# AdrienWohrer/diff-icp

Measured on AMD Instinct MI355X. Metric: PSR iterations/sec + kernel-sum HBM GB/s, 100k-pt 3D, 1/2/4/8 MI355X, higher is better.
Workload: dtype f32

## Files before the change

diff-icp_amd/csrc/lddmm_sym_pk.hpp:

```cpp
#pragma once
#include "lddmm_sym.hpp"
#include "packed.hpp"

namespace dicp {

template <int D>
struct CutBox {
  float lo[D], hi[D];
};
__device__ __forceinline__ float cut_uniform(float x) {
  return __builtin_bit_cast(float, __builtin_amdgcn_readfirstlane(__builtin_bit_cast(int, x)));
}
__device__ __forceinline__ float nan_min(float a, float b) { return (b < a || b != b) ? b : a; }
__device__ __forceinline__ float nan_max(float a, float b) { return (b > a || b != b) ? b : a; }
template <int D>
__device__ __forceinline__ void cut_load(const float* __restrict__ boxes, int s, CutBox<D>& b) {
#pragma unroll
  for (int d = 0; d < D; ++d) {
    b.lo[d] = boxes[(int64_t)s * (2 * D) + d];
    b.hi[d] = boxes[(int64_t)s * (2 * D) + D + d];
  }
}
template <int D, int N>
__device__ __forceinline__ void cut_row_box(const float* __restrict__ boxes, int s0, int nB, CutBox<D>& r) {
#pragma unroll
  for (int d = 0; d < D; ++d) r.lo[d] = __builtin_huge_valf(), r.hi[d] = -__builtin_huge_valf();
#pragma unroll
  for (int k = 0; k < N; ++k) {
    if (s0 + k >= nB) break;
    CutBox<D> b;
    cut_load<D>(boxes, s0 + k, b);
#pragma unroll
    for (int d = 0; d < D; ++d) r.lo[d] = nan_min(r.lo[d], b.lo[d]), r.hi[d] = nan_max(r.hi[d], b.hi[d]);
  }
#pragma unroll
  for (int d = 0; d < D; ++d) r.lo[d] = cut_uniform(r.lo[d]), r.hi[d] = cut_uniform(r.hi[d]);
}
template <int D, int N>
__device__ __forceinline__ unsigned cut_mask(const float* __restrict__ boxes, const CutBox<D>& r, int B, int nB,
                                             float T) {
  unsigned m = 0;
#pragma unroll
  for (int h = 0; h < N; ++h) {
    const int s = B * N + h;
    if (s >= nB) break;
    CutBox<D> c;
    cut_load<D>(boxes, s, c);
    float gap2 = 0.f;
#pragma unroll
    for (int d = 0; d < D; ++d) {
      const float a = r.lo[d] - c.hi[d], b = c.lo[d] - r.hi[d];
      float g = a > b ? a : b;
      g = g > 0.f ? g : 0.f;
      gap2 = fmaf(g, g, gap2);
    }
    if (gap2 > T) m |= 1u << h;
  }
  return (unsigned)__builtin_amdgcn_readfirstlane((int)m);
}

template <int D>
__global__ __launch_bounds__(256) void pair_boxes_kernel(Args a, int64_t M, int nB, float* __restrict__ boxes) {
  const int s = (int)blockIdx.x * 4 + (int)(threadIdx.x >> 6), l = threadIdx.x & 63;
  if (s >= nB) return;
  const int64_t i = (int64_t)s * kCutTile + l;
  float lo[D], hi[D];
  bool bad = false;
  if (i < M) {
    float c[D];
    ld_coord<D>(a, a.c0, i, c);
#pragma unroll
    for (int d = 0; d < D; ++d) {
      lo[d] = hi[d] = c[d];
      bad = bad || !(fabsf(c[d]) < __builtin_huge_valf());
    }
  } else {
#pragma unroll
    for (int d = 0; d < D; ++d) lo[d] = __builtin_huge_valf(), hi[d] = -__builtin_huge_valf();
  }
#pragma unroll
  for (int off = 32; off > 0; off >>= 1) {
#pragma unroll
    for (int d = 0; d < D; ++d) {
      lo[d] = fminf(lo[d], __shfl_xor(lo[d], off, 64));
      hi[d] = fmaxf(hi[d], __shfl_xor(hi[d], off, 64));
    }
  }
  const bool anybad = __any(bad);
  if (l < 2 * D) {
    float v = 0.f;
#pragma unroll
    for (int d = 0; d < D; ++d) {
      if (l == d) v = lo[d];
      if (l == D + d) v = hi[d];
    }
    boxes[(int64_t)s * (2 * D) + l] = anybad ? __builtin_nanf("") : v;
  }
}
template <int D>
int launch_pair_boxes(const Args& a, int64_t M, float* boxes, hipStream_t st) {
  if (M <= 0) return DICP_OK;
  const int nB = cut_tiles(M);
  pair_boxes_kernel<D><<<dim3((unsigned)((nB + 3) / 4)), dim3(256), 0, st>>>(a, M, nB, boxes);
  return check_launch("pair_boxes");
}

#ifndef DICP_SYMBWD_SCALAR_CT
#define DICP_SYMBWD_SCALAR_CT 1
#endif
template <int D, bool GQ = true, bool B0 = false, bool GT = true, bool RAW = false>
struct SymBwdPk {
  using S = SymBwd<D>;
  static constexpr int W = GQ ? 2 * D : D;
  static constexpr int kMaxWaves = 4;
#ifndef DICP_SYMBWD_PK_REC3
#define DICP_SYMBWD_PK_REC3 1
#endif
  static constexpr bool kRec3 = DICP_SYMBWD_PK_REC3 && D == 3;
  static constexpr int kPlanes = kRec3 ? 5 : S::CW;
  static constexpr bool kDupW = kRec3;
  __host__ __device__ static constexpr int slot(int i) { return kRec3 ? (i / 3) * 4 + i % 3 : i; }
  __device__ static void colvec(const float* rec, f2* cv) {
#pragma unroll
    for (int i = 0; i < 5 * D; ++i) cv[i] = splat(rec[i]);
    if constexpr (kDupW) {
#pragma unroll
      for (int m = 0; m < 5; ++m) cv[3 * m + 2] = f2{rec[3 * m + 2], rec[4 * S::CW + m]};
    }
  }
  struct Prm {
    float gt, c;
    float nc, s2;
  };
  __device__ static Prm params(const Args& a, const Scal& sc) {
    const float cs = sc.aux1 / a.scale;
    return Prm{sc.aux0 * cs, cs, sc.nc, RAW ? sc.s : kS2};
  }
  struct Row2 {
    f2 q[D], p[D], b[D], ia_a[D], gp[D];
  };
  __device__ static void pack(const typename S::Row& r0, const typename S::Row& r1, Row2& r) {
// ... 66 lines not shown
      t.cKzb = (splat(c) * zb) * t.K;
    } else {
      f2 zb = t.z[0] * (r.b[0] - bj[0]);
#pragma unroll
      for (int d = 1; d < D; ++d) zb = pk_fma(t.z[d], r.b[d] - bj[d], zb);
      t.cKzb = (splat(c) * zb) * t.K;
    }
  }
  __device__ static void pair_row(const Prm& prm, const Row2& r, const float* rec, f2* acc) {
    const float gt = prm.gt;
    f2 cv[5 * D];
    colvec(rec, cv);
    Shared t;
    shared_terms(prm, r, cv, t);
    const f2* pj = cv + D;
    const f2* aj = cv + 2 * D;
#pragma unroll
    for (int d = 0; d < D; ++d) {
      const f2 ka = GT ? pk_fma(splat(-gt), t.z[d], aj[d]) : aj[d];
      if constexpr (B0)
        acc[d] = pk_fma(t.K, ka, acc[d]);
      else
        acc[d] = pk_fma(t.cKzb, pj[d], pk_fma(t.K, ka, acc[d]));
      if constexpr (GQ) acc[D + d] = pk_fma(t.K, pk_fma(t.w, t.z[d], -t.u[d]), acc[D + d]);
    }
  }
  __device__ static void pair_sym(const Prm& prm, const Row2& r, const float* rec, f2* acc, float* ct) {
    const float gt = prm.gt;
    f2 cv[5 * D];
    colvec(rec, cv);
    Shared t;
    shared_terms(prm, r, cv, t);
    const f2* pj = cv + D;
    const f2* aj = cv + 2 * D;
    if constexpr (!GT) {
#pragma unroll
      for (int d = 0; d < D; ++d) {
        if constexpr (B0)
          acc[d] = pk_fma(t.K, aj[d], acc[d]);
        else
          acc[d] = pk_fma(t.cKzb, pj[d], pk_fma(t.K, aj[d], acc[d]));
#if DICP_SYMBWD_SCALAR_CT
        float cg = fmaf(t.K.x, r.ia_a[d].x, t.K.y * r.ia_a[d].y);
        if constexpr (!B0) cg = fmaf(t.cKzb.x, r.p[d].x, fmaf(t.cKzb.y, r.p[d].y, cg));
        ct[d] = cg;
#else
        const f2 cg = B0 ? t.K * r.ia_a[d] : pk_fma(t.cKzb, r.p[d], t.K * r.ia_a[d]);
        ct[d] = cg.x + cg.y;
#endif
        if constexpr (GQ) {
          const f2 e = pk_fma(t.w, t.z[d], -t.u[d]);
#if DICP_SYMBWD_SCALAR_CT
          acc[D + d] = pk_fma(t.K, e, acc[D + d]);
          ct[D + d] = -fmaf(t.K.x, e.x, t.K.y * e.y);
#else
          const f2 Ke = t.K * e;
          acc[D + d] = acc[D + d] + Ke;
          ct[D + d] = -(Ke.x + Ke.y);
#endif
        }
      }
      return;
    }
#pragma unroll
    for (int d = 0; d < D; ++d) {
      const f2 tt = pk_fma(splat(gt), t.z[d], r.ia_a[d]);
      if constexpr (B0) {
        acc[d] = pk_fma(t.K, pk_fma(splat(-gt), t.z[d], aj[d]), acc[d]);
        const f2 cg = t.K * tt;
        ct[d] = cg.x + cg.y;
      } else {
        acc[d] = pk_fma(t.cKzb, pj[d], pk_fma(t.K, pk_fma(splat(-gt), t.z[d], aj[d]), acc[d]));
        const f2 cg = pk_fma(t.cKzb, r.p[d], t.K * tt);
        ct[d] = cg.x + cg.y;
      }
      if constexpr (GQ) {
        const f2 e = pk_fma(t.w, t.z[d], -t.u[d]);
        const f2 Ke = t.K * e;
        acc[D + d] = acc[D + d] + Ke;
        ct[D + d] = -(Ke.x + Ke.y);
      }
    }
  }
  __device__ static void pair_sym4(const Prm& prm, const Row2& r0, const Row2& r1, const float* rec,
                                   f2* acc0, f2* acc1, float* ct) {
    const float gt = prm.gt;
    f2 cv[5 * D];
    colvec(rec, cv);
    Shared t0, t1;
    shared_terms(prm, r0, cv, t0);
    shared_terms(prm, r1, cv, t1);
    const f2* pj = cv + D;
    const f2* aj = cv + 2 * D;
#pragma unroll
    for (int d = 0; d < D; ++d) {
      const f2 ka0 = GT ? pk_fma(splat(-gt), t0.z[d], aj[d]) : aj[d];
      const f2 ka1 = GT ? pk_fma(splat(-gt), t1.z[d], aj[d]) : aj[d];
      const f2 tt0 = GT ? pk_fma(splat(gt), t0.z[d], r0.ia_a[d]) : r0.ia_a[d];
      const f2 tt1 = GT ? pk_fma(splat(gt), t1.z[d], r1.ia_a[d]) : r1.ia_a[d];
      f2 cg;
      if constexpr (B0) {
        acc0[d] = pk_fma(t0.K, ka0, acc0[d]);
        acc1[d] = pk_fma(t1.K, ka1, acc1[d]);
        cg = pk_fma(t1.K, tt1, t0.K * tt0);
      } else {
        acc0[d] = pk_fma(t0.cKzb, pj[d], pk_fma(t0.K, ka0, acc0[d]));
        acc1[d] = pk_fma(t1.cKzb, pj[d], pk_fma(t1.K, ka1, acc1[d]));
        cg = pk_fma(t1.cKzb, r1.p[d], pk_fma(t1.K, tt1, pk_fma(t0.cKzb, r0.p[d], t0.K * tt0)));
      }
      ct[d] = cg.x + cg.y;
      if constexpr (GQ) {
        const f2 e0 = pk_fma(t0.w, t0.z[d], -t0.u[d]);
        const f2 e1 = pk_fma(t1.w, t1.z[d], -t1.u[d]);
        const f2 Ke0 = t0.K * e0;
        acc0[D + d] = acc0[D + d] + Ke0;
        acc1[D + d] = pk_fma(t1.K, e1, acc1[D + d]);
        const f2 cs = pk_fma(t1.K, e1, Ke0);
        ct[D + d] = -(cs.x + cs.y);
      }
    }
  }
};

template <class P, class = void>
struct rec_layout {
  static constexpr int kPlanes = P::S::CW;
  static constexpr bool kDupW = false;
  __host__ __device__ static constexpr int slot(int i) { return i; }
};
template <class P>
struct rec_layout<P, std::void_t<decltype(P::kPlanes)>> {
  static constexpr int kPlanes = P::kPlanes;
  static constexpr bool kDupW = P::kDupW;
  __host__ __device__ static constexpr int slot(int i) { return P::slot(i); }
};
template <class P>
__host__ __device__ constexpr int plane_width(int m) {
  if (rec_layout<P>::kDupW) return 4;
  int w = 0;
  for (int i = 0; i < P::S::kUsed; ++i)
    if (rec_layout<P>::slot(i) / 4 == m && rec_layout<P>::slot(i) % 4 + 1 > w) w = rec_layout<P>::slot(i) % 4 + 1;
  return w;
}

#ifndef DICP_SYMBWD_PK_WMIN
#define DICP_SYMBWD_PK_WMIN 1
#endif
#ifndef DICP_SYMBWD_PK_WMAX
#define DICP_SYMBWD_PK_WMAX 4
#endif
#ifndef DICP_SYMBWD_PK_PREFETCH
#define DICP_SYMBWD_PK_PREFETCH 0
#endif
#ifndef DICP_SYMBWD_PK_UNROLL
#define DICP_SYMBWD_PK_UNROLL 2
#endif
template <class P>
__device__ __forceinline__ void sym_pk_body(Args a, Scal sc, int64_t M, int nG, int L,
                                            float* __restrict__ slab, int64_t slot_stride, int qoff,
                                            int qstride, unsigned bx, unsigned by) {
  using S = typename P::S;
  using LY = rec_layout<P>;
  constexpr int CW = S::CW, NP = LY::kPlanes, W = P::W;
  __shared__ float4 planes[2][NP][kSymG];
  __shared__ float colacc[kSymQ][kSymG][W];
  if (sc.dev0 != nullptr) sc.aux0 = sc.dev0[0];
  const typename P::Prm prm = P::params(a, sc);

// ... 108 lines not shown
#pragma unroll
        for (int k = 0; k < W; ++k) cacc[k] = rol1(cacc[k]);
      } else if (diag) {
#pragma unroll 2
        for (int k2 = 0; k2 < 64; ++k2) {
          const int col = h * 64 + ((l + k2) & 63);
          float rec[4 * CW + NP];
          ldrec(col, rec);
          P::pair_row(prm, row, rec, racc);
        }
      }
#pragma unroll
      for (int k = 0; k < W; ++k) colacc[wv][h * 64 + l][k] = cacc[k];
    }
    __syncthreads();
    if (tid < kSymG) {
      const int64_t j = (int64_t)B * kSymG + tid;
      if (j < M) {
        float* dst = slab + (int64_t)Q * slot_stride + j * W;
#pragma unroll
        for (int k = 0; k < W; ++k)
          dst[k] = ((colacc[0][tid][k] + colacc[1][tid][k]) + colacc[2][tid][k]) + colacc[3][tid][k];
      }
    }
    __syncthreads();
    buf ^= 1;
  }
#pragma unroll
  for (int r = 0; r < 2; ++r) {
    if (!rv[r]) continue;
    float* dst = slab + (int64_t)(Q + 1 + kc) * slot_stride + ri[r] * W;
#pragma unroll
    for (int k = 0; k < W; ++k) dst[k] = r == 0 ? racc[k].x : racc[k].y;
  }
}

#ifndef DICP_SYMBWD4_UNROLL
#define DICP_SYMBWD4_UNROLL 2
#endif
#ifndef DICP_SYMBWD4_WMIN
#define DICP_SYMBWD4_WMIN 1
#endif
template <class P, int DC = 0>
__device__ __forceinline__ void sym_pk4_body(Args a, Scal sc, int64_t M, int nG, int L,
                                             float* __restrict__ slab, int64_t slot_stride, int qoff,
                                             int qstride, unsigned bx, unsigned by,
                                             const float* __restrict__ boxes = nullptr, float T = 0.f) {
  using S = typename P::S;
  using LY = rec_layout<P>;
  constexpr int G = kSymG4;
  constexpr int CW = S::CW, NP = LY::kPlanes, W = P::W;
  __shared__ float4 planes[2][NP][G];
  __shared__ float colacc[kSymQ][G][W];
  if (sc.dev0 != nullptr) sc.aux0 = sc.dev0[0];
  const typename P::Prm prm = P::params(a, sc);

  const int Q = qoff + qstride * (int)by, kc = (int)bx;
  const int B0 = kSymQ * Q + kc * L;
  if (B0 >= nG) return;
  const int B1 = min(B0 + L, nG);
  const int tid = threadIdx.x, wv = tid >> 6, l = tid & 63;
  const int A = kSymQ * Q + wv;

  typename P::Row2 row[2];
  int64_t ri[4];
  bool rv[4];
  {
    typename S::Row r4[4];
#pragma unroll
    for (int r = 0; r < 4; ++r) {
      ri[r] = (int64_t)A * G + r * 64 + l;
      rv[r] = A < nG && ri[r] < M;
      S::load_row(a, sc, rv[r] ? ri[r] : 0, rv[r], r4[r]);
    }
    P::pack(r4[0], r4[1], row[0]);
    P::pack(r4[2], r4[3], row[1]);
  }
  f2 racc[2][W];
#pragma unroll
  for (int h = 0; h < 2; ++h)
#pragma unroll
    for (int k = 0; k < W; ++k) racc[h][k] = splat(0.f);

  CutBox<(DC > 0 ? DC : 1)> rbox;
  const int nB = cut_tiles(M);
  if constexpr (DC > 0) cut_row_box<DC, G / 64>(boxes, __builtin_amdgcn_readfirstlane(A) * (G / 64), nB, rbox);

  auto stage = [&](int B, int buf) {
    const int64_t j = (int64_t)B * G + tid;
    float rec[4 * CW], ph[4 * NP];
    S::load_col(a, sc, j < M ? j : 0, j < M, rec);
#pragma unroll
    for (int k = 0; k < 4 * NP; ++k) ph[k] = 0.f;
#pragma unroll
    for (int i = 0; i < S::kUsed; ++i) ph[LY::slot(i)] = rec[i];
    if constexpr (LY::kDupW) {
#pragma unroll
      for (int m = 0; m < NP; ++m) ph[4 * m + 3] = ph[4 * m + 2];
    }
#pragma unroll
    for (int m = 0; m < NP; ++m)
      planes[buf][m][tid] = make_float4(ph[4 * m], ph[4 * m + 1], ph[4 * m + 2], ph[4 * m + 3]);
  };

  int buf = 0;
  auto ldrec = [&](int col, float* rec) {
    float ph[4 * NP];
#pragma unroll
    for (int m = 0; m < NP; ++m) {
      const int w = plane_width<P>(m);
      const float* src = reinterpret_cast<const float*>(&planes[buf][m][col]);
      if (w == 4) {
        const float4 v = *reinterpret_cast<const float4*>(src);
        ph[4 * m] = v.x, ph[4 * m + 1] = v.y, ph[4 * m + 2] = v.z, ph[4 * m + 3] = v.w;
      } else if (w == 3) {
        const float3 v = *reinterpret_cast<const float3*>(src);
        ph[4 * m] = v.x, ph[4 * m + 1] = v.y, ph[4 * m + 2] = v.z, ph[4 * m + 3] = 0.f;
      } else if (w == 2) {
        const float2 v = *reinterpret_cast<const float2*>(src);
        ph[4 * m] = v.x, ph[4 * m + 1] = v.y, ph[4 * m + 2] = ph[4 * m + 3] = 0.f;
      } else {
        ph[4 * m] = src[0], ph[4 * m + 1] = ph[4 * m + 2] = ph[4 * m + 3] = 0.f;
      }
    }
#pragma unroll
    for (int i = 0; i < 4 * CW; ++i) rec[i] = i < S::kUsed ? ph[LY::slot(i)] : 0.f;
#pragma unroll
    for (int m = 0; m < NP; ++m) rec[4 * CW + m] = LY::kDupW ? ph[4 * m + 3] : 0.f;
  };
  stage(B0, 0);
  __syncthreads();
  for (int B = B0; B < B1; ++B) {
    if (B + 1 < B1) stage(B + 1, buf ^ 1);
    const bool sym = A < B;
    const bool diag = A == B;
    unsigned far = 0;
    if constexpr (DC > 0) {
      if (sym) far = cut_mask<DC, G / 64>(boxes, rbox, B, nB, T);
    }
#pragma unroll 1
    for (int h = 0; h < G / 64; ++h) {
      float cacc[W];
#pragma unroll
      for (int k = 0; k < W; ++k) cacc[k] = 0.f;
      if (sym && !((far >> h) & 1u)) {
#pragma unroll DICP_SYMBWD4_UNROLL
        for (int k2 = 0; k2 < 64; ++k2) {
          const int col = h * 64 + ((l + k2) & 63);
          float rec[4 * CW + NP];
          ldrec(col, rec);
          float ct[W];
          P::pair_sym4(prm, row[0], row[1], rec, racc[0], racc[1], ct);
#pragma unroll
          for (int k = 0; k < W; ++k) cacc[k] = rol1(cacc[k]) + ct[k];
        }
#pragma unroll
        for (int k = 0; k < W; ++k) cacc[k] = rol1(cacc[k]);
      } else if (diag) {
#pragma unroll 2
        for (int k2 = 0; k2 < 64; ++k2) {
          const int col = h * 64 + ((l + k2) & 63);
          float rec[4 * CW + NP];
          ldrec(col, rec);
          P::pair_row(prm, row[0], rec, racc[0]);
          P::pair_row(prm, row[1], rec, racc[1]);
        }
      }
#pragma unroll
      for (int k = 0; k < W; ++k) colacc[wv][h * 64 + l][k] = cacc[k];
    }
    __syncthreads();
    {
      const int64_t j = (int64_t)B * G + tid;
      if (j < M) {
        float* dst = slab + (int64_t)Q * slot_stride + j * W;
#pragma unroll
        for (int k = 0; k < W; ++k)
          dst[k] = ((colacc[0][tid][k] + colacc[1][tid][k]) + colacc[2][tid][k]) + colacc[3][tid][k];
      }
    }
    __syncthreads();
    buf ^= 1;
  }
#pragma unroll
  for (int r = 0; r < 4; ++r) {
    if (!rv[r]) continue;
    float* dst = slab + (int64_t)(Q + 1 + kc) * slot_stride + ri[r] * W;
    const f2* ra = racc[r >> 1];
#pragma unroll
    for (int k = 0; k < W; ++k) dst[k] = (r & 1) == 0 ? ra[k].x : ra[k].y;
  }
}

template <int D, bool GQ, bool B0, bool GT, bool RAW>
__global__ __launch_bounds__(256) __attribute__((amdgpu_waves_per_eu(DICP_SYMBWD4_WMIN, 4))) void sym_bwd_pk4_kernel(
    Args a, Scal sc, int64_t M, int nG, int L, float* __restrict__ slab, int64_t slot_stride, int qoff,
    int qstride) {
  sym_pk4_body<SymBwdPk<D, GQ, B0, GT, RAW>>(a, sc, M, nG, L, slab, slot_stride, qoff, qstride, blockIdx.x,
                                             blockIdx.y);
}

template <int D, bool GQ, bool B0, bool GT, bool RAW>
__global__ __launch_bounds__(256) __attribute__((amdgpu_waves_per_eu(DICP_SYMBWD_PK_WMIN, DICP_SYMBWD_PK_WMAX))) void sym_bwd_pk_kernel(
    Args a, Scal sc, int64_t M, int nG, int L, float* __restrict__ slab, int64_t slot_stride, int qoff,
    int qstride) {
  sym_pk_body<SymBwdPk<D, GQ, B0, GT, RAW>>(a, sc, M, nG, L, slab, slot_stride, qoff, qstride, blockIdx.x,
                                            blockIdx.y);
}

template <int D, bool GQ, bool B0, bool GT>
__global__ __launch_bounds__(256) __attribute__((amdgpu_waves_per_eu(DICP_SYMBWD4_WMIN, 4))) void sym_bwd_pk4_cut_kernel(
    Args a, Scal sc, int64_t M, int nG, int L, float* __restrict__ slab, int64_t slot_stride,
    const float* __restrict__ boxes, float T) {
  sym_pk4_body<SymBwdPk<D, GQ, B0, GT, false>, D>(a, sc, M, nG, L, slab, slot_stride, 0, 1, blockIdx.x, blockIdx.y,
                                                  boxes, T);
}

template <int D, bool GQ, bool B0, bool GT, bool RAW>
__global__ __launch_bounds__(256) __attribute__((amdgpu_waves_per_eu(DICP_SYMBWD_PK_WMIN, DICP_SYMBWD_PK_WMAX))) void sym_bwd_pk_batch_kernel(
    BatchTab<SymEntry> t) {
  const SymEntry& e = t.e[blockIdx.z];
  if (blockIdx.x >= e.gx || blockIdx.y >= e.gy) return;
  sym_pk_body<SymBwdPk<D, GQ, B0, GT, RAW>>(e.a, e.sc, e.M, e.nG, e.L, e.slab, e.slot_stride, e.qoff, e.qstride,
                                            blockIdx.x, blockIdx.y);
}
template <int D, bool GQ, bool B0, bool GT, bool RAW>
__global__ __launch_bounds__(256) __attribute__((amdgpu_waves_per_eu(DICP_SYMBWD4_WMIN, 4))) void sym_bwd_pk4_batch_kernel(
    BatchTab<SymEntry> t) {
  const SymEntry& e = t.e[blockIdx.z];
  if (blockIdx.x >= e.gx || blockIdx.y >= e.gy) return;
  sym_pk4_body<SymBwdPk<D, GQ, B0, GT, RAW>>(e.a, e.sc, e.M, e.nG, e.L, e.slab, e.slot_stride, e.qoff, e.qstride,
                                             blockIdx.x, blockIdx.y);
}
template <int D, bool GQ, bool B0, bool GT, bool RAW>
int sym_bwd_pk_batch_flush(const std::vector<const void*>& es, hipStream_t st) {
  return batch_launch<SymEntry>(sym_bwd_pk_batch_kernel<D, GQ, B0, GT, RAW>, es, st, "sym_bwd_pk");
}
// ... 183 lines not shown
      if (DIV) acc[2 * D + d] = pk_fma(K, z[d], acc[2 * D + d]);
    }
  }
  __device__ static void pair_sym(const Prm&, const Row2& r, const float* rec, f2* acc, float* ct) {
    f2 z[D];
    f2 r2 = splat(0.f);
#pragma unroll
    for (int d = 0; d < D; ++d) {
      z[d] = r.q[d] - splat(rec[d]);
      r2 = pk_fma(z[d], z[d], r2);
    }
    const f2 K = f2{fast_exp2(-r2.x), fast_exp2(-r2.y)};
    const float* pj = rec + D;
    f2 pp = r.p[0] * splat(pj[0]);
#pragma unroll
    for (int d = 1; d < D; ++d) pp = pk_fma(r.p[d], splat(pj[d]), pp);
    const f2 Kpp = K * pp;
#pragma unroll
    for (int d = 0; d < D; ++d) {
      acc[d] = pk_fma(K, splat(pj[d]), acc[d]);
      acc[D + d] = pk_fma(Kpp, z[d], acc[D + d]);
      if (DIV) acc[2 * D + d] = pk_fma(K, z[d], acc[2 * D + d]);
      ct[d] = fmaf(K.x, r.p[d].x, K.y * r.p[d].y);
      ct[D + d] = -fmaf(Kpp.x, z[d].x, Kpp.y * z[d].y);
      if (DIV) ct[2 * D + d] = -fmaf(K.x, z[d].x, K.y * z[d].y);
    }
  }
};

template <int D, bool DIV>
struct SymFwdPk4 {
  using S = SymFwd<D, DIV>;
  static constexpr int W = S::W;
  static constexpr bool kRec3 = D == 3;
  static constexpr int kPlanes = kRec3 ? 2 : S::CW;
  static constexpr bool kDupW = kRec3;
  __host__ __device__ static constexpr int slot(int i) { return kRec3 ? (i / 3) * 4 + i % 3 : i; }
  struct Prm {};
  __device__ static Prm params(const Args&, const Scal&) { return Prm{}; }
  using Row2 = typename SymFwdPk<D, DIV>::Row2;
  __device__ static void pack(const typename S::Row& r0, const typename S::Row& r1, Row2& r) {
    SymFwdPk<D, DIV>::pack(r0, r1, r);
  }
  __device__ static void colvec(const float* rec, f2* cv) {
#pragma unroll
    for (int i = 0; i < 2 * D; ++i) cv[i] = splat(rec[i]);
    if constexpr (kDupW) {
#pragma unroll
      for (int m = 0; m < 2; ++m) cv[3 * m + 2] = f2{rec[3 * m + 2], rec[4 * S::CW + m]};
    }
  }
  struct Sh {
    f2 z[D];
    f2 K, Kpp;
  };
  __device__ static void shared(const Row2& r, const f2* cv, Sh& t) {
    f2 r2 = splat(0.f);
#pragma unroll
    for (int d = 0; d < D; ++d) {
      t.z[d] = r.q[d] - cv[d];
      r2 = pk_fma(t.z[d], t.z[d], r2);
    }
    t.K = f2{fast_exp2(-r2.x), fast_exp2(-r2.y)};
    f2 pp = r.p[0] * cv[D];
#pragma unroll
    for (int d = 1; d < D; ++d) pp = pk_fma(r.p[d], cv[D + d], pp);
    t.Kpp = t.K * pp;
  }
  __device__ static void row_side(const Sh& t, const f2* cv, f2* acc) {
#pragma unroll
    for (int d = 0; d < D; ++d) {
      acc[d] = pk_fma(t.K, cv[D + d], acc[d]);
      acc[D + d] = pk_fma(t.Kpp, t.z[d], acc[D + d]);
      if (DIV) acc[2 * D + d] = pk_fma(t.K, t.z[d], acc[2 * D + d]);
    }
  }
  __device__ static void pair_row(const Prm&, const Row2& r, const float* rec, f2* acc) {
    f2 cv[2 * D];
    colvec(rec, cv);
    Sh t;
    shared(r, cv, t);
    row_side(t, cv, acc);
  }
  __device__ static void pair_sym4(const Prm&, const Row2& r0, const Row2& r1, const float* rec, f2* acc0,
                                   f2* acc1, float* ct) {
    f2 cv[2 * D];
    colvec(rec, cv);
    Sh t0, t1;
    shared(r0, cv, t0);
    shared(r1, cv, t1);
    row_side(t0, cv, acc0);
    row_side(t1, cv, acc1);
#pragma unroll
    for (int d = 0; d < D; ++d) {
      const f2 cV = pk_fma(t1.K, r1.p[d], t0.K * r0.p[d]);
      ct[d] = cV.x + cV.y;
      const f2 cG = pk_fma(t1.Kpp, t1.z[d], t0.Kpp * t0.z[d]);
      ct[D + d] = -(cG.x + cG.y);
      if (DIV) {
        const f2 cZ = pk_fma(t1.K, t1.z[d], t0.K * t0.z[d]);
        ct[2 * D + d] = -(cZ.x + cZ.y);
      }
    }
  }
};

template <int NRP>
constexpr int sym_fwd_group() { return 128 * NRP; }
constexpr int kSymG8 = 512;
template <int D, bool DIV, int NRP>
struct SymFwdPkN {
  using P4 = SymFwdPk4<D, DIV>;
  using S = typename P4::S;
  static constexpr int W = S::W;
  using Row2 = typename P4::Row2;
  using Sh = typename P4::Sh;
  __device__ static void pair_sym(const Row2* r, const float* rec, f2 (*acc)[W], float* ct) {
    f2 cv[2 * D];
    P4::colvec(rec, cv);
    f2 cV[D], cG[D], cZ[D];
#pragma unroll
    for (int h = 0; h < NRP; ++h) {
      Sh t;
      P4::shared(r[h], cv, t);
      P4::row_side(t, cv, acc[h]);
#pragma unroll
      for (int d = 0; d < D; ++d) {
        cV[d] = h == 0 ? t.K * r[h].p[d] : pk_fma(t.K, r[h].p[d], cV[d]);
        cG[d] = h == 0 ? t.Kpp * t.z[d] : pk_fma(t.Kpp, t.z[d], cG[d]);
        if (DIV) cZ[d] = h == 0 ? t.K * t.z[d] : pk_fma(t.K, t.z[d], cZ[d]);
      }
    }
#pragma unroll
    for (int d = 0; d < D; ++d) {
      ct[d] = cV[d].x + cV[d].y;
      ct[D + d] = -(cG[d].x + cG[d].y);
      if (DIV) ct[2 * D + d] = -(cZ[d].x + cZ[d].y);
    }
  }
  __device__ static void pair_row(const Row2& r, const float* rec, f2* acc) {
    P4::pair_row(typename P4::Prm{}, r, rec, acc);
  }
};

#ifndef DICP_SYMFWD8_WPE
#define DICP_SYMFWD8_WPE 1
#endif
template <int D, bool DIV, int NRP, bool CUT = false>
__device__ __forceinline__ void sym_fwd_pkn_body(const Args& a, const Scal& sc, int64_t M, int nG, int L,
                                                 float* __restrict__ slab, int64_t slot_stride, unsigned bx,
                                                 unsigned by, const float* __restrict__ boxes = nullptr,
                                                 float T = 0.f) {
  using P = SymFwdPkN<D, DIV, NRP>;
  using P4 = SymFwdPk4<D, DIV>;
  using S = typename P::S;
  using LY = rec_layout<P4>;
  constexpr int G = sym_fwd_group<NRP>(), NR = 2 * NRP;
  constexpr int CW = S::CW, NP = LY::kPlanes, W = P::W;
  __shared__ float4 planes[2][NP][G];
  __shared__ float colacc[kSymQ][64][W];

  const int Q = (int)by, kc = (int)bx;
  const int B0 = kSymQ * Q + kc * L;
  if (B0 >= nG) return;
  const int B1 = min(B0 + L, nG);
  const int tid = threadIdx.x, wv = tid >> 6, l = tid & 63;
  const int A = kSymQ * Q + wv;

  typename P::Row2 row[NRP];
  const int64_t rbase = (int64_t)A * G + l;
  {
    typename S::Row rr[NR];
#pragma unroll
    for (int r = 0; r < NR; ++r) {
      const int64_t ri = rbase + r * 64;
      const bool rv = A < nG && ri < M;
      S::load_row(a, sc, rv ? ri : 0, rv, rr[r]);
    }
#pragma unroll
    for (int h = 0; h < NRP; ++h) P4::pack(rr[2 * h], rr[2 * h + 1], row[h]);
  }
  f2 racc[NRP][W];
#pragma unroll
  for (int h = 0; h < NRP; ++h)
#pragma unroll
    for (int k = 0; k < W; ++k) racc[h][k] = splat(0.f);

  CutBox<D> rbox;
  const int nB = cut_tiles(M);
  if constexpr (CUT) cut_row_box<D, G / 64>(boxes, __builtin_amdgcn_readfirstlane(A) * (G / 64), nB, rbox);

  auto stage = [&](int B, int buf) {
#pragma unroll
    for (int u = 0; u < (G + 255) / 256; ++u) {
      const int c = u * 256 + tid;
      if (G % 256 != 0 && c >= G) break;
      const int64_t j = (int64_t)B * G + c;
      float rec[4 * CW], ph[4 * NP];
      S::load_col(a, sc, j < M ? j : 0, j < M, rec);
#pragma unroll
      for (int k = 0; k < 4 * NP; ++k) ph[k] = 0.f;
#pragma unroll
      for (int i = 0; i < S::kUsed; ++i) ph[LY::slot(i)] = rec[i];
      if constexpr (LY::kDupW) {
#pragma unroll
        for (int m = 0; m < NP; ++m) ph[4 * m + 3] = ph[4 * m + 2];
      }
#pragma unroll
      for (int m = 0; m < NP; ++m)
        planes[buf][m][c] = make_float4(ph[4 * m], ph[4 * m + 1], ph[4 * m + 2], ph[4 * m + 3]);
    }
  };
  int buf = 0;
  auto ldrec = [&](int col, float* rec) {
    float ph[4 * NP];
#pragma unroll
    for (int m = 0; m < NP; ++m) {
      const float4 v = planes[buf][m][col];
      ph[4 * m] = v.x, ph[4 * m + 1] = v.y, ph[4 * m + 2] = v.z, ph[4 * m + 3] = v.w;
    }
#pragma unroll
    for (int i = 0; i < 4 * CW; ++i) rec[i] = i < S::kUsed ? ph[LY::slot(i)] : 0.f;
#pragma unroll
    for (int m = 0; m < NP; ++m) rec[4 * CW + m] = LY::kDupW ? ph[4 * m + 3] : 0.f;
  };
  stage(B0, 0);
  __syncthreads();
  for (int B = B0; B < B1; ++B) {
    if (B + 1 < B1) stage(B + 1, buf ^ 1);
    const bool sym = A < B;
    const bool diag = A == B;
    unsigned far = 0;
    if constexpr (CUT) {
      if (sym) far = cut_mask<D, G / 64>(boxes, rbox, B, nB, T);
    }
#pragma unroll 1
    for (int h = 0; h < G / 64; ++h) {
      {
        float cacc[W];
#pragma unroll
        for (int k = 0; k < W; ++k) cacc[k] = 0.f;
        if (sym && !((far >> h) & 1u)) {
#pragma unroll 1
          for (int k2 = 0; k2 < 64; ++k2) {
            const int col = h * 64 + ((l + k2) & 63);
            float rec[4 * CW + NP];
            ldrec(col, rec);
            float ct[W];
            P::pair_sym(row, rec, racc, ct);
#pragma unroll
            for (int k = 0; k < W; ++k) cacc[k] = rol1(cacc[k]) + ct[k];
          }
#pragma unroll
          for (int k = 0; k < W; ++k) cacc[k] = rol1(cacc[k]);
        } else if (diag) {
#pragma unroll 1
          for (int k2 = 0; k2 < 64; ++k2) {
            const int col = h * 64 + ((l + k2) & 63);
            float rec[4 * CW + NP];
            ldrec(col, rec);
#pragma unroll
            for (int r = 0; r < NRP; ++r) P::pair_row(row[r], rec, racc[r]);
          }
        }
#pragma unroll
        for (int k = 0; k < W; ++k) colacc[wv][l][k] = cacc[k];
      }
      __syncthreads();
      {
        const int64_t j0 = (int64_t)B * G + h * 64;
        float* dst = slab + (int64_t)Q * slot_stride + j0 * W;
        for (int e = tid; e < 64 * W; e += 256) {
          const int c = e / W, k = e - c * W;
          if (j0 + c < M) dst[e] = ((colacc[0][c][k] + colacc[1][c][k]) + colacc[2][c][k]) + colacc[3][c][k];
        }
      }
      __syncthreads();
    }
    buf ^= 1;
  }
#pragma unroll
  for (int r = 0; r < NR; ++r) {
    const int64_t ri = rbase + r * 64;
    if (!(A < nG && ri < M)) continue;
    float* dst = slab + (int64_t)(Q + 1 + kc) * slot_stride + ri * W;
    const f2* ra = racc[r >> 1];
#pragma unroll
    for (int k = 0; k < W; ++k) dst[k] = (r & 1) == 0 ? ra[k].x : ra[k].y;
  }
}

template <int D, bool DIV, int NRP>
__global__ __launch_bounds__(256) __attribute__((amdgpu_waves_per_eu(NRP == 4 ? DICP_SYMFWD8_WPE : 3, 4))) void sym_fwd_pkn_kernel(
    Args a, Scal sc, int64_t M, int nG, int L, float* __restrict__ slab, int64_t slot_stride) {
  sym_fwd_pkn_body<D, DIV, NRP>(a, sc, M, nG, L, slab, slot_stride, blockIdx.x, blockIdx.y);
}
template <int D, bool DIV, int NRP>
__global__ __launch_bounds__(256) __attribute__((amdgpu_waves_per_eu(NRP == 4 ? DICP_SYMFWD8_WPE : 3, 4))) void sym_fwd_pkn_cut_kernel(
    Args a, Scal sc, int64_t M, int nG, int L, float* __restrict__ slab, int64_t slot_stride,
    const float* __restrict__ boxes, float T) {
  sym_fwd_pkn_body<D, DIV, NRP, true>(a, sc, M, nG, L, slab, slot_stride, blockIdx.x, blockIdx.y, boxes, T);
}
template <int D, bool DIV, int NRP>
__global__ __launch_bounds__(256) __attribute__((amdgpu_waves_per_eu(NRP == 4 ? DICP_SYMFWD8_WPE : 3, 4))) void sym_fwd_pkn_batch_kernel(
    BatchTab<SymEntry> t) {
  const SymEntry& e = t.e[blockIdx.z];
  if (blockIdx.x >= e.gx || blockIdx.y >= e.gy) return;
  sym_fwd_pkn_body<D, DIV, NRP>(e.a, e.sc, e.M, e.nG, e.L, e.slab, e.slot_stride, blockIdx.x, blockIdx.y);
}
template <int D, bool DIV, int NRP>
int sym_fwd_pkn_batch_flush(const std::vector<const void*>& es, hipStream_t st) {
  return batch_launch<SymEntry>(sym_fwd_pkn_batch_kernel<D, DIV, NRP>, es, st, "sym_fwd_pkn");
}

template <int D, bool DIV, int NRP = 4>
int launch_sym_fwdn(const Args& a, const Scal& sc, int64_t M, const Outs& o, void* ws, size_t wsb,
                    hipStream_t st, bool zs) {
  using S = SymFwd<D, DIV>;
  constexpr int G = sym_fwd_group<NRP>();
  if (M <= 0) return DICP_OK;
  const SymGeom g = sym_geom(M, 1, G, 4, NRP == 4 ? kSymFwd8WgMin : kSymFwd6WgMin);
  const size_t need = sym_ws_bytes(M, S::W);
  if (ws == nullptr || wsb < need) {
    set_error("ode_self_fwd(sym6/8): workspace too small (%zu < %zu bytes)", wsb, need);
    return DICP_ERR_WORKSPACE;
  }
  if (o.ptr[0] == nullptr || (zs && (!DIV || o.ptr[3] == nullptr))) {
    set_error("ode_self_fwd(sym6/8): v is required, zs needs the divergence sums");
    return DICP_ERR_INVALID;
  }
  float* slab = reinterpret_cast<float*>(ws);
  const int64_t stride = M * S::W;
  const dim3 grid((unsigned)g.Kmax, (unsigned)g.nQ), mg((unsigned)((M + 255) / 256));
  const float ia = 1.f / a.scale;
// ... 64 lines not shown
```

Baseline: 0.5887.

## Refine distance cutoff to per-row-pair bounding boxes with specialized partial kernels

Row tiles used to be tested against column subtiles with a single bounding box for the whole row group. Now each packed row pair gets its own box and its own bit in the far mask. A compile-time-dispatched specialization of the pair kernels then computes only the active row pairs, so interactions beyond the cutoff are skipped at finer granularity. The cost is more mask computation, more template instantiations (code size, instruction cache, register pressure) and a runtime branch dispatch per subtile.

After: 0.6066, median of 6. +3.0%, better.

```diff
diff --git a/diff-icp_amd/csrc/lddmm_sym_pk.hpp b/diff-icp_amd/csrc/lddmm_sym_pk.hpp
--- a/diff-icp_amd/csrc/lddmm_sym_pk.hpp
+++ b/diff-icp_amd/csrc/lddmm_sym_pk.hpp
@@ -57,6 +57,49 @@
     if (gap2 > T) m |= 1u << h;
   }
   return (unsigned)__builtin_amdgcn_readfirstlane((int)m);
+}
+
+#ifndef DICP_CUT_ROWPAIR
+#define DICP_CUT_ROWPAIR 1
+#endif
+constexpr bool kCutRowPair = DICP_CUT_ROWPAIR != 0;
+template <int D, int NRP>
+__device__ __forceinline__ void cut_rowpair_boxes(const float* __restrict__ boxes, int s0, int nB, CutBox<D>* r) {
+#pragma unroll
+  for (int k = 0; k < NRP; ++k) cut_row_box<D, 2>(boxes, s0 + 2 * k, nB, r[k]);
+}
+template <int D, int N, int NRP>
+__device__ __forceinline__ unsigned cut_mask_rowpair(const float* __restrict__ boxes, const CutBox<D>* r, int B,
+                                                     int nB, float T) {
+  static_assert(N * NRP <= 32, "one mask word");
+  unsigned m = 0;
+#pragma unroll
+  for (int h = 0; h < N; ++h) {
+    const int s = B * N + h;
+    if (s >= nB) break;
+    CutBox<D> c;
+    cut_load<D>(boxes, s, c);
+#pragma unroll
+    for (int k = 0; k < NRP; ++k) {
+      float gap2 = 0.f;
+#pragma unroll
+      for (int d = 0; d < D; ++d) {
+        const float a = r[k].lo[d] - c.hi[d], b = c.lo[d] - r[k].hi[d];
+        float g = a > b ? a : b;
+        g = g > 0.f ? g : 0.f;
+        gap2 = fmaf(g, g, gap2);
+      }
+      if (gap2 > T) m |= 1u << (h * NRP + k);
+    }
+  }
+  return (unsigned)__builtin_amdgcn_readfirstlane((int)m);
+}
+template <unsigned ACT, class F>
+__device__ __forceinline__ void cut_dispatch(unsigned act, F&& f) {
+  if (act == ACT)
+    f(std::integral_constant<unsigned, ACT>{});
+  else if constexpr (ACT > 1u)
+    cut_dispatch<ACT - 1u>(act, f);
 }
 
 template <int D>
@@ -289,8 +332,45 @@
       }
     }
   }
+  template <unsigned ACT = 3u>
   __device__ static void pair_sym4(const Prm& prm, const Row2& r0, const Row2& r1, const float* rec,
                                    f2* acc0, f2* acc1, float* ct) {
+    static_assert(ACT >= 1u && ACT <= 3u, "mask of active row pairs");
+    if constexpr (ACT != 3u) {
+      constexpr bool kFirst = ACT == 1u;
+      const Row2& r = kFirst ? r0 : r1;
+      f2* acc = kFirst ? acc0 : acc1;
+      const float gt = prm.gt;
+      f2 cv[5 * D];
+      colvec(rec, cv);
+      Shared t;
+      shared_terms(prm, r, cv, t);
+      const f2* pj = cv + D;
+      const f2* aj = cv + 2 * D;
+#pragma unroll
+      for (int d = 0; d < D; ++d) {
+        const f2 ka = GT ? pk_fma(splat(-gt), t.z[d], aj[d]) : aj[d];
+        const f2 tt = GT ? pk_fma(splat(gt), t.z[d], r.ia_a[d]) : r.ia_a[d];
+        f2 cg = pk_fma(t.K, tt, splat(0.f));
+        if constexpr (B0) {
+          acc[d] = pk_fma(t.K, ka, acc[d]);
+        } else {
+          acc[d] = pk_fma(t.cKzb, pj[d], pk_fma(t.K, ka, acc[d]));
+          cg = pk_fma(t.cKzb, r.p[d], cg);
+        }
+        ct[d] = cg.x + cg.y;
+        if constexpr (GQ) {
+          const f2 e = pk_fma(t.w, t.z[d], -t.u[d]);
+          if constexpr (kFirst)
+            acc[D + d] = acc[D + d] + t.K * e;
+          else
+            acc[D + d] = pk_fma(t.K, e, acc[D + d]);
+          const f2 cs = pk_fma(t.K, e, splat(0.f));
+          ct[D + d] = -(cs.x + cs.y);
+        }
+      }
+      return;
+    }
     const float gt = prm.gt;
     f2 cv[5 * D];
     colvec(rec, cv);
@@ -565,9 +645,13 @@
 #pragma unroll
     for (int k = 0; k < W; ++k) racc[h][k] = splat(0.f);
 
-  CutBox<(DC > 0 ? DC : 1)> rbox;
+  constexpr bool kRowPair = DC > 0 && kCutRowPair;
+  CutBox<(DC > 0 ? DC : 1)> rbox, rpbox[2];
   const int nB = cut_tiles(M);
-  if constexpr (DC > 0) cut_row_box<DC, G / 64>(boxes, __builtin_amdgcn_readfirstlane(A) * (G / 64), nB, rbox);
+  if constexpr (kRowPair)
+    cut_rowpair_boxes<DC, 2>(boxes, __builtin_amdgcn_readfirstlane(A) * (G / 64), nB, rpbox);
+  else if constexpr (DC > 0)
+    cut_row_box<DC, G / 64>(boxes, __builtin_amdgcn_readfirstlane(A) * (G / 64), nB, rbox);
 
   auto stage = [&](int B, int buf) {
     const int64_t j = (int64_t)B * G + tid;
@@ -619,23 +703,45 @@
     const bool diag = A == B;
     unsigned far = 0;
     if constexpr (DC > 0) {
-      if (sym) far = cut_mask<DC, G / 64>(boxes, rbox, B, nB, T);
+      if (sym) {
+        if constexpr (kRowPair)
+          far = cut_mask_rowpair<DC, G / 64, 2>(boxes, rpbox, B, nB, T);
+        else
+          far = cut_mask<DC, G / 64>(boxes, rbox, B, nB, T);
+      }
     }
 #pragma unroll 1
     for (int h = 0; h < G / 64; ++h) {
       float cacc[W];
 #pragma unroll
       for (int k = 0; k < W; ++k) cacc[k] = 0.f;
-      if (sym && !((far >> h) & 1u)) {
+      unsigned act = 3u;
+      if constexpr (kRowPair) act = ~(far >> (2 * h)) & 3u;
+      if (sym && (kRowPair ? act != 0u : !((far >> h) & 1u))) {
+        if constexpr (kRowPair) {
+          cut_dispatch<3u>(act, [&](auto ac) {
 #pragma unroll DICP_SYMBWD4_UNROLL
-        for (int k2 = 0; k2 < 64; ++k2) {
-          const int col = h * 64 + ((l + k2) & 63);
-          float rec[4 * CW + NP];
-          ldrec(col, rec);
-          float ct[W];
-          P::pair_sym4(prm, row[0], row[1], rec, racc[0], racc[1], ct);
-#pragma unroll
-          for (int k = 0; k < W; ++k) cacc[k] = rol1(cacc[k]) + ct[k];
+            for (int k2 = 0; k2 < 64; ++k2) {
+              const int col = h * 64 + ((l + k2) & 63);
+              float rec[4 * CW + NP];
+              ldrec(col, rec);
+              float ct[W];
+              P::template pair_sym4<decltype(ac)::value>(prm, row[0], row[1], rec, racc[0], racc[1], ct);
+#pragma unroll
+              for (int k = 0; k < W; ++k) cacc[k] = rol1(cacc[k]) + ct[k];
+            }
+          });
+        } else {
+#pragma unroll DICP_SYMBWD4_UNROLL
+          for (int k2 = 0; k2 < 64; ++k2) {
+            const int col = h * 64 + ((l + k2) & 63);
+            float rec[4 * CW + NP];
+            ldrec(col, rec);
+            float ct[W];
+            P::pair_sym4(prm, row[0], row[1], rec, racc[0], racc[1], ct);
+#pragma unroll
+            for (int k = 0; k < W; ++k) cacc[k] = rol1(cacc[k]) + ct[k];
+          }
         }
 #pragma unroll
         for (int k = 0; k < W; ++k) cacc[k] = rol1(cacc[k]);
@@ -985,8 +1091,30 @@
     shared(r, cv, t);
     row_side(t, cv, acc);
   }
+  template <unsigned ACT = 3u>
   __device__ static void pair_sym4(const Prm&, const Row2& r0, const Row2& r1, const float* rec, f2* acc0,
                                    f2* acc1, float* ct) {
+    static_assert(ACT >= 1u && ACT <= 3u, "mask of active row pairs");
+    if constexpr (ACT != 3u) {
+      const Row2& r = ACT == 1u ? r0 : r1;
+      f2 cv[2 * D];
+      colvec(rec, cv);
+      Sh t;
+      shared(r, cv, t);
+      row_side(t, cv, ACT == 1u ? acc0 : acc1);
+#pragma unroll
+      for (int d = 0; d < D; ++d) {
+        const f2 cV = pk_fma(t.K, r.p[d], splat(0.f));
+        ct[d] = cV.x + cV.y;
+        const f2 cG = pk_fma(t.Kpp, t.z[d], splat(0.f));
+        ct[D + d] = -(cG.x + cG.y);
+        if (DIV) {
+          const f2 cZ = pk_fma(t.K, t.z[d], splat(0.f));
+          ct[2 * D + d] = -(cZ.x + cZ.y);
+        }
+      }
+      return;
+    }
     f2 cv[2 * D];
     colvec(rec, cv);
     Sh t0, t1;
@@ -1018,20 +1146,28 @@
   static constexpr int W = S::W;
   using Row2 = typename P4::Row2;
   using Sh = typename P4::Sh;
+  static constexpr unsigned kAll = (1u << NRP) - 1u;
+  template <unsigned ACT = kAll>
   __device__ static void pair_sym(const Row2* r, const float* rec, f2 (*acc)[W], float* ct) {
+    static_assert(ACT >= 1u && ACT <= kAll, "mask of active row pairs");
     f2 cv[2 * D];
     P4::colvec(rec, cv);
     f2 cV[D], cG[D], cZ[D];
+    if constexpr (ACT != kAll) {
+#pragma unroll
+      for (int d = 0; d < D; ++d) cV[d] = cG[d] = cZ[d] = splat(0.f);
+    }
 #pragma unroll
     for (int h = 0; h < NRP; ++h) {
+      if (!((ACT >> h) & 1u)) continue;
       Sh t;
       P4::shared(r[h], cv, t);
       P4::row_side(t, cv, acc[h]);
 #pragma unroll
       for (int d = 0; d < D; ++d) {
-        cV[d] = h == 0 ? t.K * r[h].p[d] : pk_fma(t.K, r[h].p[d], cV[d]);
-        cG[d] = h == 0 ? t.Kpp * t.z[d] : pk_fma(t.Kpp, t.z[d], cG[d]);
-        if (DIV) cZ[d] = h == 0 ? t.K * t.z[d] : pk_fma(t.K, t.z[d], cZ[d]);
+        cV[d] = (ACT == kAll && h == 0) ? t.K * r[h].p[d] : pk_fma(t.K, r[h].p[d], cV[d]);
+        cG[d] = (ACT == kAll && h == 0) ? t.Kpp * t.z[d] : pk_fma(t.Kpp, t.z[d], cG[d]);
+        if (DIV) cZ[d] = (ACT == kAll && h == 0) ? t.K * t.z[d] : pk_fma(t.K, t.z[d], cZ[d]);
       }
     }
 #pragma unroll
@@ -1089,9 +1225,13 @@
 #pragma unroll
     for (int k = 0; k < W; ++k) racc[h][k] = splat(0.f);
 
-  CutBox<D> rbox;
+  constexpr bool kRowPair = CUT && kCutRowPair;
+  CutBox<D> rbox, rpbox[NRP];
   const int nB = cut_tiles(M);
-  if constexpr (CUT) cut_row_box<D, G / 64>(boxes, __builtin_amdgcn_readfirstlane(A) * (G / 64), nB, rbox);
+  if constexpr (kRowPair)
+    cut_rowpair_boxes<D, NRP>(boxes, __builtin_amdgcn_readfirstlane(A) * (G / 64), nB, rpbox);
+  else if constexpr (CUT)
+    cut_row_box<D, G / 64>(boxes, __builtin_amdgcn_readfirstlane(A) * (G / 64), nB, rbox);
 
   auto stage = [&](int B, int buf) {
 #pragma unroll
@@ -1135,7 +1275,12 @@
     const bool diag = A == B;
     unsigned far = 0;
     if constexpr (CUT) {
-      if (sym) far = cut_mask<D, G / 64>(boxes, rbox, B, nB, T);
+      if (sym) {
+        if constexpr (kRowPair)
+          far = cut_mask_rowpair<D, G / 64, NRP>(boxes, rpbox, B, nB, T);
+        else
+          far = cut_mask<D, G / 64>(boxes, rbox, B, nB, T);
+      }
     }
 #pragma unroll 1
     for (int h = 0; h < G / 64; ++h) {
@@ -1143,16 +1288,33 @@
         float cacc[W];
 #pragma unroll
         for (int k = 0; k < W; ++k) cacc[k] = 0.f;
-        if (sym && !((far >> h) & 1u)) {
+        unsigned act = P::kAll;
+        if constexpr (kRowPair) act = ~(far >> (NRP * h)) & P::kAll;
+        if (sym && (kRowPair ? act != 0u : !((far >> h) & 1u))) {
+          if constexpr (kRowPair) {
+            cut_dispatch<P::kAll>(act, [&](auto ac) {
 #pragma unroll 1
-          for (int k2 = 0; k2 < 64; ++k2) {
-            const int col = h * 64 + ((l + k2) & 63);
-            float rec[4 * CW + NP];
-            ldrec(col, rec);
-            float ct[W];
-            P::pair_sym(row, rec, racc, ct);
-#pragma unroll
-            for (int k = 0; k < W; ++k) cacc[k] = rol1(cacc[k]) + ct[k];
+              for (int k2 = 0; k2 < 64; ++k2) {
+                const int col = h * 64 + ((l + k2) & 63);
+                float rec[4 * CW + NP];
+                ldrec(col, rec);
+                float ct[W];
+                P::template pair_sym<decltype(ac)::value>(row, rec, racc, ct);
+#pragma unroll
+                for (int k = 0; k < W; ++k) cacc[k] = rol1(cacc[k]) + ct[k];
+              }
+            });
+          } else {
+#pragma unroll 1
+            for (int k2 = 0; k2 < 64; ++k2) {
+              const int col = h * 64 + ((l + k2) & 63);
+              float rec[4 * CW + NP];
+              ldrec(col, rec);
+              float ct[W];
+              P::pair_sym(row, rec, racc, ct);
+#pragma unroll
+              for (int k = 0; k < W; ++k) cacc[k] = rol1(cacc[k]) + ct[k];
+            }
           }
 #pragma unroll
           for (int k = 0; k < W; ++k) cacc[k] = rol1(cacc[k]);
```
